# sebastianffx/stainlib

Hardware: AMD Instinct MI355X
Metric: 1024x1024 H&E tiles/sec normalized (Macenko) (higher is better)
Workload: dtype f32; 1 GPU; configs[1]: batch of 512 tiles 1024x1024x3 uint8 per GPU, Macenko transform (fit once outside the timed region), tiles resident in HBM; tiles_per_gpu=512, failed_tiles=0

## Files before the change

stainlib_amd/csrc/stats_finish.hpp:

```cpp
#pragma once
#include "stats_selection.hpp"
#include "stats_sweeps.hpp"

namespace sl {

struct SampleAngleKey {
    const uint32_t* sample; TabView tab; float V[6]; int cps_log2; int P; float ylimf;
    __device__ __forceinline__ float operator()(int b) const {
        if (sample_absent(b, cps_log2, P)) return nan_f();
        return of_word(sample[b]);
    }
    __device__ __forceinline__ float of_word(uint32_t s) const {
        const uint32_t r = s & 255u, g = (s >> 8) & 255u, bl = (s >> 16) & 255u;
        const bool tissue = is_tissue_f(tab.gam(r), tab.gam(g), tab.gam(bl), ylimf);
        const float k = angle_key(V, tab.odf(r), tab.odf(g), tab.odf(bl));
        return tissue ? k : nan_f();
    }
    __device__ __forceinline__ bool present(int b, int n_sample) const { return b < n_sample && !sample_absent(b, cps_log2, P); }
};
struct SampleConcKey {
    const uint32_t* sample; TabView tab; LassoK L; int cps_log2; int P; int col;
    __device__ __forceinline__ void both(int b, float& c1, float& c2) const {
        if (sample_absent(b, cps_log2, P)) { c1 = c2 = nan_f(); return; }
        of_word(sample[b], c1, c2);
// ... 100 lines not shown
    __syncthreads();
}

struct Census { uint32_t n_below, n_in, omin, omax; };
template <class KeyAt>
__device__ __noinline__ Census wg_bracket_census(int n, KeyAt key_at, float lo, float hi, SelScratch& S) {
    if (threadIdx.x == 0) { S.misc[4] = 0xffffffffu; S.misc[5] = 0; S.misc[6] = 0; S.misc[7] = 0; }
    __syncthreads();
    const uint32_t olo = f2ord(lo), ohi = f2ord(hi);
    uint32_t mn = 0xffffffffu, mx = 0, nb = 0, ni = 0;
    wg_for_each_key(n, key_at, [&](uint32_t o) {
        nb += o < olo ? 1u : 0u;
        if (o >= olo && o <= ohi) { ++ni; mn = min(mn, o); mx = max(mx, o); }
    });
    for (int o = 32; o > 0; o >>= 1) {
        mn = min(mn, (uint32_t)__shfl_xor((int)mn, o, 64));
        mx = max(mx, (uint32_t)__shfl_xor((int)mx, o, 64));
        nb += __shfl_xor((int)nb, o, 64);
        ni += __shfl_xor((int)ni, o, 64);
    }
    if ((threadIdx.x & 63) == 0) { atomicMin(&S.misc[4], mn); atomicMax(&S.misc[5], mx); atomicAdd(&S.misc[6], nb); atomicAdd(&S.misc[7], ni); }
    __syncthreads();
    const Census c{S.misc[6], S.misc[7], S.misc[4], S.misc[5]};
    __syncthreads();
    return c;
}

template <class TileKeyAt>
__device__ __forceinline__ void stage_order_stats(const float* cand, uint32_t n_in, uint32_t cap_list, bool complete, float lo, float hi,
                                                  long long lt, int P, const TileKeyAt& tile_key_at, uint32_t n,
                                                  long long k, float& xa, float& xb, int& fallbacks, SelScratch& S) {
    const long long k2 = (k + 1 < (long long)n) ? k + 1 : k;
    const bool covered = complete && k >= lt && k2 < lt + (long long)n_in;
    if (covered && lo == hi) {
        xa = xb = lo;
    } else if (covered && n_in <= cap_list) {
        wg_select_pair_small((int)n_in, CandKey{cand}, (uint32_t)(k - lt), xa, xb, S);
        if (k2 == k) xb = xa;
    } else {
        const Census c = wg_bracket_census(P, tile_key_at, lo, hi, S);
        if (c.n_in > 0 && c.omin == c.omax && k >= (long long)c.n_below && k2 < (long long)c.n_below + (long long)c.n_in) {
            xa = xb = ord2f(c.omin);
        } else {
            wg_select_pair(P, tile_key_at, (uint32_t)k, xa, xb, S);
            if (k2 == k) xb = xa;
        }
        fallbacks += 1;
    }
}

struct PickScale { float lo[2], sc[2]; };
__device__ __forceinline__ int pick_bin(float k, float lo, float sc) { return min(511, max(0, (int)((k - lo) * sc))); }

__device__ __forceinline__ void wg_pick2(const float* cand0, const float* cand1, const uint32_t* n_in, const bool* want, const uint32_t* krel,
                                         const PickScale& ps, float* xa , float* xb , bool* done , SelScratch& S) {
    const int tid = threadIdx.x, lane = tid & 63, wave = tid >> 6;
#pragma unroll
    for (int b = 0; b < 2; ++b)
        if (wave == b && want[b]) wave_locate(S.hist + 512 * b, 512, krel[b], &S.misc[16 + 3 * b], lane);
    if (tid < 2) { S.misc[24 + tid] = 0; S.misc[26 + tid] = 0xffffffffu; }
    __syncthreads();
    uint32_t bin[2], below[2], cnt[2];
#pragma unroll
    for (int b = 0; b < 2; ++b) { bin[b] = S.misc[16 + 3 * b]; below[b] = S.misc[17 + 3 * b]; cnt[b] = S.misc[18 + 3 * b]; done[b] = want[b] && cnt[b] <= 512u && cnt[b] > 0u; }
    __syncthreads();
    float* list = reinterpret_cast<float*>(S.hist);
#pragma unroll
    for (int b = 0; b < 2; ++b) {
        if (!done[b]) continue;
        const float* cand = b ? cand1 : cand0;
        const int n = (int)n_in[b];
        constexpr int U = 4;
        const int bd = blockDim.x;
        uint32_t best = 0xffffffffu;
        float kn[U];
#pragma unroll
        for (int u = 0; u < U; ++u) { const int i = tid + u * bd; kn[u] = as_global(cand)[i < n ? i : 0]; }
        for (int i0 = tid; i0 < n; i0 += U * bd) {
            float k[U];
#pragma unroll
            for (int u = 0; u < U; ++u) {
                k[u] = kn[u];
                const int i = i0 + (U + u) * bd;
                kn[u] = as_global(cand)[i < n ? i : 0];
            }
#pragma unroll
            for (int u = 0; u < U; ++u) {
                if (i0 + u * bd >= n) continue;
                const int kb = pick_bin(k[u], ps.lo[b], ps.sc[b]);
                if (kb == (int)bin[b]) { const uint32_t pos = atomicAdd(&S.misc[24 + b], 1u); if (pos < 512u) list[512 * b + pos] = k[u]; }
                else if (kb > (int)bin[b]) best = min(best, f2ord(k[u]));
            }
        }
        for (int o = 32; o > 0; o >>= 1) best = min(best, (uint32_t)__shfl_xor((int)best, o, 64));
        if (lane == 0 && best != 0xffffffffu) atomicMin(&S.misc[26 + b], best);
    }
    __syncthreads();
    if (tid < 4) S.misc[28 + tid] = 0;
    __syncthreads();
#pragma unroll
    for (int b = 0; b < 2; ++b) {
        if (!done[b]) continue;
        const uint32_t m = cnt[b], ra = krel[b] - below[b];
        if ((uint32_t)tid < m) {
            const float me = list[512 * b + tid];
            uint32_t r = 0;
            for (uint32_t j = 0; j < m; ++j) {
                const float o = list[512 * b + j];
                r += (o < me || (o == me && j < (uint32_t)tid)) ? 1u : 0u;
            }
            if (r == ra) S.misc[28 + 2 * b] = __float_as_uint(me);
            if (r == ra + 1) S.misc[29 + 2 * b] = __float_as_uint(me);
        }
    }
    __syncthreads();
#pragma unroll
    for (int b = 0; b < 2; ++b) {
        if (!done[b]) continue;
        xa[b] = __uint_as_float(S.misc[28 + 2 * b]);
        const bool same_bin = krel[b] - below[b] + 1 < cnt[b];
        const uint32_t nx = S.misc[26 + b];
        xb[b] = same_bin ? __uint_as_float(S.misc[29 + 2 * b]) : (nx != 0xffffffffu ? ord2f(nx) : xa[b]);
    }
    __syncthreads();
}

template <bool TWO_COLS, class TileKeyAt>
__device__ __forceinline__ void stage_pick2(const float* cand0, const float* cand1, const uint32_t* n_in, uint32_t cap_list, bool complete,
                                            const float* lo, const float* hi, const long long* lt, int P, TileKeyAt tile_key_at, uint32_t n,
                                            const long long* k, const PickScale& ps, float* res , int& fallbacks, SelScratch& S) {
    bool fast[2], has2[2];
    uint32_t krel[2];
#pragma unroll
    for (int b = 0; b < 2; ++b) {
        const long long k2 = (k[b] + 1 < (long long)n) ? k[b] + 1 : k[b];
        has2[b] = k2 != k[b];
        const bool covered = complete && k[b] >= lt[b] && k2 < lt[b] + (long long)n_in[b];
        fast[b] = covered && lo[b] < hi[b] && n_in[b] <= cap_list;
        krel[b] = fast[b] ? (uint32_t)(k[b] - lt[b]) : 0u;
    }
    float xa[2] = {0, 0}, xb[2] = {0, 0};
    bool done[2] = {false, false};
    if (fast[0] | fast[1]) wg_pick2(cand0, cand1, n_in, fast, krel, ps, xa, xb, done, S);
#pragma unroll
    for (int b = 0; b < 2; ++b) {
        if (done[b]) {
            if (!has2[b]) xb[b] = xa[b];
        } else {
            if constexpr (TWO_COLS) tile_key_at.col = b;
            stage_order_stats(b ? cand1 : cand0, n_in[b], cap_list, complete, lo[b], hi[b], lt[b], P, tile_key_at, n, k[b], xa[b], xb[b], fallbacks, S);
        }
        res[2 * b] = xa[b]; res[2 * b + 1] = xb[b];
    }
}

__device__ __noinline__ void raw_flush(uint32_t buf_lds, uint32_t n, uint32_t* dst, unsigned int* head, uint32_t cap) {
#if defined(__HIP_DEVICE_COMPILE__)
    SL_LDS const uint32_t* buf = (SL_LDS const uint32_t*)buf_lds;
#else
    const uint32_t* buf = nullptr;
#endif
    const int lane = threadIdx.x & 63;
    uint32_t base = 0;
    if (lane == 0) base = atomicAdd(head, n);
    base = __builtin_amdgcn_readfirstlane(base);
    for (uint32_t i = lane; i < n; i += 64)
        if (base + i < cap) as_global(dst)[base + i] = buf[i];
}

struct RawSink {
    uint32_t buf;
    uint32_t n;
    uint32_t* dst;
    unsigned int* head;
    unsigned int* overflow;
    uint32_t cap;
    uint32_t stage_cap;
    __device__ __forceinline__ void flush(int) {
        if (n != 0) raw_flush(buf, n, dst, head, cap);
        n = 0;
    }
    __device__ __forceinline__ void put(unsigned long long m, const Chunk& ch, int px, int lane) {
        put_value(m, chunk_pixel(ch, px) & 0xffffffu, lane);
    }
    __device__ __forceinline__ void put_value(unsigned long long m, uint32_t value, int lane) {
        const uint32_t cnt = (uint32_t)__popcll(m);
        if (__builtin_expect(n + cnt > stage_cap, 0)) flush(lane);
        const uint32_t rank = __builtin_amdgcn_mbcnt_hi((uint32_t)(m >> 32), __builtin_amdgcn_mbcnt_lo((uint32_t)m, 0u));
#if defined(__HIP_DEVICE_COMPILE__)
        uint32_t sbase;
        asm("s_lshl2_add_u32 %0, %1, %2" : "=s"(sbase) : "s"(n), "s"(buf) : "scc");
        const uint32_t addr = sbase + 4u * rank;
        unsigned long long saved;
        asm volatile("s_mov_b64 %0, exec\n\ts_mov_b64 exec, %1\n\tds_write_b32 %2, %3\n\ts_mov_b64 exec, %0"
                     : "=&s"(saved) : "s"(m), "v"(addr), "v"(value) : "memory");
#else
        (void)rank; (void)value;
#endif
        n += cnt;
    }
};


// ... 16 lines not shown
    __device__ __forceinline__ TabView view() const { return TabView{base, 8u, 4u, 0u}; }
};
__device__ __forceinline__ void fin_tab_build(RowTab& tab) {
    float2* p = reinterpret_cast<float2*>(tab.e);
    float2 e = make_float2(0.0f, 0.0f);
    if (threadIdx.x < 256) e = p[threadIdx.x * 32];
    __syncthreads();
    if (threadIdx.x < 256) p[threadIdx.x] = e;
    __syncthreads();
}

template <int NT>
__device__ __forceinline__ void fin_tab_expand(RowTab& tab) {
    float2* p = reinterpret_cast<float2*>(tab.e);
    constexpr int PER = 256 * 32 / NT;
    float2 e[PER];
#pragma unroll
    for (int j = 0; j < PER; ++j) e[j] = p[threadIdx.x / 32 + j * (NT / 32)];
    __syncthreads();
#pragma unroll
    for (int j = 0; j < PER; ++j) p[threadIdx.x + j * NT] = e[j];
    __syncthreads();
}

struct WordAngleKey {
    FinTab T; float V[6]; float ylimf;
    __device__ __forceinline__ void of_word(uint32_t s, float& k0, float& k1, bool& valid) const {
        const float2 er = T.gam_odf(T.addr(s, 0)), eg = T.gam_odf(T.addr(s, 1)), eb = T.gam_odf(T.addr(s, 2));
        valid = is_tissue_f(er.x, eg.x, eb.x, ylimf);
        k0 = k1 = angle_key(V, er.y, eg.y, eb.y);
    }
};
struct WordConcKey {
    FinTab T; LassoK L;
    __device__ __forceinline__ void of_word(uint32_t s, float& k0, float& k1, bool& valid) const {
        lasso2(L, T.odf(T.addr(s, 0)), T.odf(T.addr(s, 1)), T.odf(T.addr(s, 2)), k0, k1);
        valid = true;
    }
};

__device__ __forceinline__ void lds_count_masked(unsigned long long m, uint32_t addr, uint32_t one) {
#if defined(__HIP_DEVICE_COMPILE__)
    unsigned long long saved;
    asm volatile("s_mov_b64 %0, exec\n\ts_mov_b64 exec, %1\n\tds_add_u32 %2, %3\n\ts_mov_b64 exec, %0"
                 : "=&s"(saved) : "s"(m), "v"(addr), "v"(one) : "memory");
#else
    (void)m; (void)addr; (void)one;
#endif
}

struct RefineOut { uint32_t n_lt[2], n_in[2], n_valid; PickScale ps; };
template <class WordKey2>
__device__ __forceinline__ RefineOut wg_refine_s(const uint32_t* raw, int n_raw, const WordKey2& key2, float lo0, float hi0, float lo1, float hi1,
                                                 float* cand0, float* cand1, uint32_t cap_list, uint32_t stage_lds, uint32_t stage_entries,
                                                 SelScratch& S) {
    const int tid = threadIdx.x, lane = tid & 63;
    if (tid < 5) S.misc[8 + tid] = 0;
    for (int i = tid; i < 1024; i += blockDim.x) S.hist[i] = 0;
    RefineOut r;
    r.ps.lo[0] = lo0; r.ps.lo[1] = lo1;
    r.ps.sc[0] = (hi0 > lo0 && lo0 > -INFINITY && hi0 < INFINITY) ? 512.0f * 0.999999f / (hi0 - lo0) : 0.0f;
    r.ps.sc[1] = (hi1 > lo1 && lo1 > -INFINITY && hi1 < INFINITY) ? 512.0f * 0.999999f / (hi1 - lo1) : 0.0f;
    __syncthreads();
    stage_lds = (uint32_t)__builtin_amdgcn_readfirstlane((int)stage_lds);
    RawSink s0{stage_lds, 0u, reinterpret_cast<uint32_t*>(cand0), &S.misc[11], nullptr, cap_list, stage_entries};
    RawSink s1{stage_lds + 4u * stage_entries, 0u, reinterpret_cast<uint32_t*>(cand1), &S.misc[12], nullptr, cap_list, stage_entries};
    const float vlo0 = in_vgpr(lo0), vhi0 = in_vgpr(hi0), vlo1 = in_vgpr(lo1), vhi1 = in_vgpr(hi1);
    const float psl0 = in_vgpr(r.ps.lo[0]), psc0 = in_vgpr(r.ps.sc[0]), psl1 = in_vgpr(r.ps.lo[1]), psc1 = in_vgpr(r.ps.sc[1]);
    const uint32_t hist_lds = lds_address(S.hist);
    uint32_t one = 1u;
    asm("" : "+v"(one));
    uint32_t lt0 = 0, lt1 = 0, nv = 0;
    constexpr int U = 4;
    const int step = (int)blockDim.x * U;
    const int last = n_raw > 0 ? n_raw - 1 : 0;
    int i0 = (tid - lane) * U;
    uint32_t wn[U];
#pragma unroll
    for (int u = 0; u < U; ++u) wn[u] = as_global(raw)[min(i0 + u * 64 + lane, last)];
    for (; i0 < n_raw; i0 += step) {
        uint32_t w[U];
#pragma unroll
        for (int u = 0; u < U; ++u) {
            w[u] = wn[u];
            wn[u] = as_global(raw)[min(i0 + step + u * 64 + lane, last)];
        }
#pragma unroll
        for (int u = 0; u < U; ++u) {
            float k0, k1;
            bool valid;
            key2.of_word(w[u], k0, k1, valid);
            const bool inb = i0 + u * 64 + lane < n_raw;
            const unsigned long long mv = __builtin_amdgcn_ballot_w64(valid) & __builtin_amdgcn_ballot_w64(inb);
            const unsigned long long l0 = __builtin_amdgcn_ballot_w64(k0 < vlo0) & mv, l1 = __builtin_amdgcn_ballot_w64(k1 < vlo1) & mv;
            const unsigned long long m0 = __builtin_amdgcn_ballot_w64(k0 <= vhi0) & ~l0 & mv, m1 = __builtin_amdgcn_ballot_w64(k1 <= vhi1) & ~l1 & mv;
            nv += (uint32_t)__popcll(mv);
            lt0 += (uint32_t)__popcll(l0);
            lt1 += (uint32_t)__popcll(l1);
            lds_count_masked(m0, hist_lds + 4u * (uint32_t)pick_bin(k0, psl0, psc0), one);
            lds_count_masked(m1, hist_lds + 2048u + 4u * (uint32_t)pick_bin(k1, psl1, psc1), one);
            s0.put_value(m0, __float_as_uint(k0), lane);
            s1.put_value(m1, __float_as_uint(k1), lane);
        }
    }
    s0.flush(lane);
    s1.flush(lane);
    if (lane == 0) { if (nv) atomicAdd(&S.misc[8], nv); if (lt0) atomicAdd(&S.misc[9], lt0); if (lt1) atomicAdd(&S.misc[10], lt1); }
    __threadfence_block();
    __syncthreads();
    r.n_lt[0] = S.misc[9]; r.n_lt[1] = S.misc[10]; r.n_in[0] = S.misc[11]; r.n_in[1] = S.misc[12]; r.n_valid = S.misc[8];
    __syncthreads();
    return r;
}

constexpr float kBoxZ = 3.6f;
template <int THREADS>
__device__ __forceinline__ void angle_brackets(const SampleAngleKey& key, int n_sample, double pct, float* lo, float* hi,
                                               SelScratch& S, float* box = nullptr, float zs = 1.0f) {
    constexpr int KPT = kMaxSample / THREADS;
    uint32_t ord[1][KPT];
#ifdef SL_DEBUG_SUBCLK
    long long bclk_t_ = wall_clock64();
#endif
    static_assert(KPT % kBrkBatch == 0, "");
#pragma unroll
    for (int j0 = 0; j0 < KPT; j0 += kBrkBatch) {
        uint32_t w[kBrkBatch];
#pragma unroll
        for (int g = 0; g < kBrkBatch; ++g) {
            const int b = (j0 + g) * THREADS + (int)threadIdx.x;
            w[g] = b < n_sample ? as_global(key.sample)[b] : 0u;
        }
#pragma unroll
        for (int g = 0; g < kBrkBatch; ++g) {
            const int b = (j0 + g) * THREADS + (int)threadIdx.x;
            const float k = key.of_word(w[g]);
            ord[0][j0 + g] = (k == k && key.present(b, n_sample)) ? f2ord(k) : kAbsent;
        }
    }
    SL_BCLK(5);
    const int set_of[2] = {0, 0};
    const double p2[2] = {100.0 - pct, pct};
    wg_brackets_regs<1, KPT, 2>(ord, set_of, p2, lo, hi, S, kBracketZ * zs);
    if (box) {
        const bool closed = (lo[0] > -INFINITY) & (hi[0] < INFINITY) & (lo[1] > -INFINITY) & (hi[1] < INFINITY);
        if (closed) {
#pragma unroll
            for (int b = 0; b < 2; ++b) {
                const float m = 0.5f * (lo[b] + hi[b]), r = (float)kBoxFrac * 0.5f * (hi[b] - lo[b]);
                box[2 * b] = m - r; box[2 * b + 1] = m + r;
            }
        } else {
            const double n = (double)S.misc[6], q = p2[0] / 100.0;
            const bool inside = n > 0.0 && floor(q * (n - 1.0) - (double)(kBoxZ * zs) * sqrt(fmax(q * (1.0 - q) * n, 0.0))) - 1.0 >= 0.0;
            float blo[2] = {-INFINITY, -INFINITY}, bhi[2] = {INFINITY, INFINITY};
            __syncthreads();
            if (inside) wg_brackets_regs<1, KPT, 2>(ord, set_of, p2, blo, bhi, S, kBoxZ * zs);
            box[0] = blo[0]; box[1] = bhi[0]; box[2] = blo[1]; box[3] = bhi[1];
        }
    }
// ... 35 lines not shown
```

stainlib_amd/csrc/stats_fused.hpp:

```cpp
#pragma once
#include "stats_phase_kernels.hpp"
#include "stats_cube.hpp"
#include "stats_twosweep.hpp"

namespace sl {

struct FusedArgs {
    const uint8_t* rgb;
    uint8_t* out;
    int n_tiles;
    int P;
    int stride_log2;
    int n_sample;
    float ylimf;
    double lam;
    double pct;
    const double* M_tgt;
    const double* maxC_tgt;
    int cap_raw, cap_list;
    uint32_t* raw;
    int cap_ang;
    uint32_t* raw_ang;
    float* cand;
    uint32_t* sample;
// ... 274 lines not shown
    const int tid = threadIdx.x;
    const TabReaderB TB = TabReaderB::make_at(FusedLds<NT>::tab);
    const int nch = (P + 3) >> 2;
    ApplyK K;
    apply_consts(sh.M, sh.maxC, M_tgt, maxC_tgt, lam, K);
    int t, c0, c1;
    fused_geometry<NT>(nch, tid, t, c0, c1);
    if (c0 >= c1) return;
    if (stream) {
        if (K.fast) apply_sweep<ALIGNED, true, TabReaderB, true>(src, dst, P, c0, c1, t, kFusedThreads, TB, K);
        else apply_sweep<ALIGNED, false, TabReaderB, true>(src, dst, P, c0, c1, t, kFusedThreads, TB, K);
    } else {
        if (K.fast) apply_sweep<ALIGNED, true, TabReaderB, false>(src, dst, P, c0, c1, t, kFusedThreads, TB, K);
        else apply_sweep<ALIGNED, false, TabReaderB, false>(src, dst, P, c0, c1, t, kFusedThreads, TB, K);
    }
}

template <int NT, bool ALIGNED>
__device__ __noinline__ void fused_sweep2_cube(FusedShared<NT>* shp, const uint8_t* src_, uint32_t* rawl_, uint32_t* rawa_, int P_, int cap_raw_, int cap_ang_,
                                               float ylimf_, int stream_) {
    FusedShared<NT>& sh = *shp;
    const uint8_t* src = uni_ptr(src_);
    uint32_t* rawl = uni_ptr(rawl_);
    uint32_t* rawa = uni_ptr(rawa_);
    const int P = __builtin_amdgcn_readfirstlane(P_), cap_raw = __builtin_amdgcn_readfirstlane(cap_raw_), stream = __builtin_amdgcn_readfirstlane(stream_);
    const int cap_ang = __builtin_amdgcn_readfirstlane(cap_ang_);
    const float ylimf = uni(ylimf_);
    const int tid = threadIdx.x, wave = tid >> 6;
    const TabReaderB TB = TabReaderB::make_at(FusedLds<NT>::tab);
    const int nch = (P + 3) >> 2;
    SelConsts K;
    for (int i = 0; i < 6; ++i) K.V[i] = in_vgpr(sh.Vf[i]);
    K.L.g12 = 0.0f;
    K.xmin = -INFINITY;
#pragma unroll
    for (int i = 0; i < 2; ++i) {
        K.u[i][0] = in_vgpr(sh.mk.u[i][0]); K.u[i][1] = in_vgpr(sh.mk.u[i][1]); K.kt[i] = in_vgpr(sh.mk.kt[i]);
        K.eps[i] = in_vgpr(sh.mk.eps[i]); K.thr[i] = in_vgpr(sh.mk.thr[i]);
    }
    K.lo0 = uni(sh.lo[0]); K.hi0 = uni(sh.hi[0]); K.lo1 = uni(sh.lo[1]); K.hi1 = uni(sh.hi[1]);
    static_assert(offsetof(FusedShared<NT>, n_ang) == offsetof(FusedShared<NT>, n_raw) + 4 && offsetof(FusedShared<NT>, n_raw) % 8 == 0, "");
    const RawDirect direct{rawl, rawa, reinterpret_cast<unsigned long long*>(&sh.n_raw), (uint32_t)cap_raw, (uint32_t)cap_ang};
    static_assert(offsetof(FusedShared<NT>, S) % 4096 == 0 && offsetof(SelScratch, hist) == 0, "the cube mask must be 4 KB aligned");
    const uint32_t bits_lds = FusedLds<NT>::hist;
    const uint32_t ring_lds = (uint32_t)__builtin_amdgcn_readfirstlane((int)(FusedLds<NT>::stage + (uint32_t)wave * FusedLds<NT>::stage_wave));
    int t, c0, c1;
    fused_geometry<NT>(nch, tid, t, c0, c1);
    if (c0 >= c1) return;
    if (stream) select_sweep_cube<ALIGNED, kFusedTrip, true>(src, P, c0, c1, t, kFusedThreads, TB, ylimf, K, bits_lds, ring_lds, direct);
    else select_sweep_cube<ALIGNED, kFusedTrip, false>(src, P, c0, c1, t, kFusedThreads, TB, ylimf, K, bits_lds, ring_lds, direct);
}

template <int NT>
__device__ SL_FINISH_ATTR int fused_finish2(FusedShared<NT>* shp, const uint8_t* src_, uint32_t* rawl_, uint32_t* rawa_, float* cand0_, float* cand1_, int P_,
                                          int cap_raw_, int cap_ang_, int cap_list_, float ylimf_, double pct_, double lam_, long long* subclk_, int ts_ = 0) {
    FusedShared<NT>& sh = *shp;
    const uint8_t* src = uni_ptr(src_);
    uint32_t* rawl = uni_ptr(rawl_);
    uint32_t* rawa = uni_ptr(rawa_);
    const int cap_ang = __builtin_amdgcn_readfirstlane(cap_ang_);
    float* cand0 = uni_ptr(cand0_);
    float* cand1 = uni_ptr(cand1_);
    const int P = __builtin_amdgcn_readfirstlane(P_), cap_raw = __builtin_amdgcn_readfirstlane(cap_raw_), cap_list = __builtin_amdgcn_readfirstlane(cap_list_);
    const float ylimf = uni(ylimf_);
    const double pct = uni_d(pct_), lam = uni_d(lam_);
    long long* subclk = uni_ptr(subclk_);
    const int ts = __builtin_amdgcn_readfirstlane(ts_);
    const int tid = threadIdx.x, wave = tid >> 6;
    int fallbacks = 0;
#ifdef SL_DEBUG_SUBCLK
#define SL_SUB(j) { __syncthreads(); if (subclk && tid == 0) subclk[(j)] = wall_clock64(); }
#else
#define SL_SUB(j)
#endif
    (void)subclk;
    const uint32_t T = (uint32_t)sh.sum[0];
    long long k[2];
    double gfrac[2];
    percentile_pos((double)T, 100.0 - pct, k[0], gfrac[0]);
    percentile_pos((double)T, pct, k[1], gfrac[1]);
    fin_tab_build(sh.tab);
    const FinTab FT{FusedLds<NT>::tab};
    const uint32_t stage_lds = FusedLds<NT>::tab + kFinTabBytes + (uint32_t)wave * fin_stage_bytes(NT);
    const uint32_t stage_entries = fin_stage_bytes(NT) / 8u;
    AngleTileKey tkey;
    tkey.src = src; tkey.tab = FT.view(); tkey.ylimf = ylimf;
    WordAngleKey rkey;
    rkey.T = FT; rkey.ylimf = ylimf;
    for (int i = 0; i < 6; ++i) { tkey.V[i] = sh.Vf[i]; rkey.V[i] = sh.Vf[i]; }
    const bool complete = sh.n_raw <= (uint32_t)cap_raw && sh.overflow == 0;
    const uint32_t n_raw = sh.n_raw < (uint32_t)cap_raw ? sh.n_raw : (uint32_t)cap_raw;
    const bool split = rawa != nullptr;
    const bool complete_a = split ? sh.n_ang <= (uint32_t)cap_ang : complete;
    const uint32_t n_a = split ? (sh.n_ang < (uint32_t)cap_ang ? sh.n_ang : (uint32_t)cap_ang) : n_raw;
    const uint32_t* lista = split ? rawa : rawl;
    const float los[2] = {sh.lo[0], sh.lo[1]}, his[2] = {sh.hi[0], sh.hi[1]};
    SL_SUB(2);
    const RefineOut ra = wg_refine_s(lista, (int)n_a, rkey, los[0], his[0], los[1], his[1], cand0, cand1, (uint32_t)cap_list, stage_lds,
                                     stage_entries, sh.S);
    SL_SUB(3);
    {
        const long long lt[2] = {(long long)ra.n_lt[0], (long long)T - (long long)ra.n_valid + (long long)ra.n_lt[1]};
        if (ts) {
            bool covered = complete_a;
#pragma unroll
            for (int b = 0; b < 2; ++b) {
                const long long k2 = (k[b] + 1 < (long long)T) ? k[b] + 1 : k[b];
                covered = covered & (k[b] >= lt[b]) & (k2 < lt[b] + (long long)ra.n_in[b]) & (ra.n_in[b] <= (uint32_t)cap_list);
            }
            if (!covered) {
                fin_tab_expand<NT>(sh.tab);
                return -1;
            }
        }
        float res[4];
        stage_pick2<false>(cand0, cand1, ra.n_in, (uint32_t)cap_list, complete_a, los, his, lt, P, tkey, T, k, ra.ps, res, fallbacks, sh.S);
        if (tid == 0) { sh.res[0] = res[0]; sh.res[1] = res[1]; sh.res[2] = res[2]; sh.res[3] = res[3]; }
        __syncthreads();
    }
    SL_SUB(5);
    if (tid < 64) {
        double M[6];
        stain_matrix_from_angles(sh.Vd, sh.res, gfrac, M, tid);
        if (tid == 0) {
            for (int i = 0; i < 6; ++i) sh.M[i] = M[i];
            if (stain_matrix_singular(M)) sh.status = SL_TILE_DEGENERATE_COV;
            const bool use = sh.status == SL_TILE_OK && complete && merged_verify(sh.mk, M, lam);
            sh.conc_done = use ? 1 : 0;
            sh.why = use ? 0 : (!sh.mk.ok ? SL_RESWEEP_NO_BOX : (!complete ? SL_RESWEEP_LIST_FULL : SL_RESWEEP_OUTSIDE_BOX));
            if (use) { LassoK L; lasso_consts(M, lam, L); sh.L = L; }
        }
    }
    __syncthreads();
    SL_SUB(6);
    if (sh.conc_done) {
        long long kc;
        double gc;
        percentile_pos((double)P, 99.0, kc, gc);
        const long long kc2 = kc + 1 < (long long)P ? kc + 1 : kc;
        WordConcKey ckey2;
        ckey2.T = FT; ckey2.L = sh.L;
        const float cl[2] = {sh.mk.L[0], sh.mk.L[1]}, chh[2] = {sh.mk.H[0], sh.mk.H[1]};
        const RefineOut rc = wg_refine_s(rawl, (int)n_raw, ckey2, cl[0], chh[0], cl[1], chh[1], cand0, cand1, (uint32_t)cap_list,
                                         stage_lds, stage_entries, sh.S);
        SL_SUB(14);
#ifdef SL_DEBUG_SUBCLK
        if (subclk && tid == 0) {
            long long* q = subclk;
            q[8] = 100ll * n_a; q[9] = 100ll * n_raw; q[10] = 100ll * (ra.n_in[0] + ra.n_in[1]); q[11] = 100ll * (rc.n_in[0] + rc.n_in[1]);
        }
#endif
        const long long n_plain = (long long)P - (long long)sh.n_raw;
        const long long clt[2] = {n_plain + rc.n_lt[0], n_plain + rc.n_lt[1]};
        bool covered = true;
#pragma unroll
        for (int col = 0; col < 2; ++col)
            covered = covered & (kc >= clt[col]) & (kc2 < clt[col] + (long long)rc.n_in[col]) & (rc.n_in[col] <= (uint32_t)cap_list);
        if (covered) {
            ConcTileKey ctk;
            ctk.src = src; ctk.tab = FT.view(); ctk.L = sh.L; ctk.col = 0;
            const long long kk[2] = {kc, kc};
            float res[4];
            stage_pick2<true>(cand0, cand1, rc.n_in, (uint32_t)cap_list, true, cl, chh, clt, P, ctk, (uint32_t)P, kk, rc.ps, res, fallbacks, sh.S);
            if (tid == 0) {
                sh.maxC[0] = np_lerp((double)res[0], (double)res[1], gc);
                sh.maxC[1] = np_lerp((double)res[2], (double)res[3], gc);
                if (!(sh.maxC[0] > 0.0) || !(sh.maxC[1] > 0.0)) sh.status = SL_TILE_ZERO_MAXC;
            }
        } else if (tid == 0) {
            sh.conc_done = 0;
            sh.why = (rc.n_in[0] > (uint32_t)cap_list || rc.n_in[1] > (uint32_t)cap_list) ? SL_RESWEEP_LIST_FULL : SL_RESWEEP_BRACKET_MISSED;
        }
        __syncthreads();
        SL_SUB(15);
    }
    fin_tab_expand<NT>(sh.tab);
    return fallbacks;
#undef SL_SUB
}

template <int NT>
__device__ __noinline__ void phase0_estimate(FusedShared<NT>* shp, int mode_) {
    FusedShared<NT>& sh = *shp;
    const int mode = __builtin_amdgcn_readfirstlane(mode_);
    double Vd[6], wv[3];
    float Vf[6];
    const int st = eigvecs_from_moments(sh.sum, Vd, Vf, wv);
    const double ns = sh.sum[0];
    const double l1 = wv[0], l2 = wv[1], l3 = wv[2] > 0.0 ? wv[2] : 0.0;
    bool ok = st == SL_TILE_OK && ns >= (double)kTsMinTissue && l2 > 1e-9 * l1 && l2 - l3 > 0.05 * l2;
    double tau = 0.0;
    if (ok) {
        tau = kTiltZ * sqrt(kClusterDeff / ns) * fmax(sqrt(l3 * l2) / (l2 - l3), sqrt(l3 * l1) / (l1 - l3));
        tau = fmax(tau, kTsMinTau);
        ok = tau <= (mode >= 2 ? kTsMaxTau : kTsAutoMaxTau);
    }
    double nd[3] = {Vd[2] * Vd[5] - Vd[4] * Vd[3], Vd[4] * Vd[1] - Vd[0] * Vd[5], Vd[0] * Vd[3] - Vd[2] * Vd[1]};
    const double nn = 1.0 / sqrt(nd[0] * nd[0] + nd[1] * nd[1] + nd[2] * nd[2]);
    if (mode == 4 && ok) {
        double b[3];
        for (int c = 0; c < 3; ++c) b[c] = Vd[2 * c + 1] + 0.05 * nd[c] * nn;
        const double nb = 1.0 / sqrt(b[0] * b[0] + b[1] * b[1] + b[2] * b[2]);
        for (int c = 0; c < 3; ++c) { Vd[2 * c + 1] = b[c] * nb; Vf[2 * c + 1] = (float)Vd[2 * c + 1]; }
        nd[0] = Vd[2] * Vd[5] - Vd[4] * Vd[3]; nd[1] = Vd[4] * Vd[1] - Vd[0] * Vd[5]; nd[2] = Vd[0] * Vd[3] - Vd[2] * Vd[1];
    }
    const double nn2 = 1.0 / sqrt(nd[0] * nd[0] + nd[1] * nd[1] + nd[2] * nd[2]);
    for (int i = 0; i < 6; ++i) { sh.ts.Vd[i] = Vd[i]; sh.Vd[i] = Vd[i]; sh.Vf[i] = Vf[i]; }
    for (int c = 0; c < 3; ++c) { sh.ts.nd[c] = nd[c] * nn2; sh.ts.fn[c] = (float)(nd[c] * nn2); }
    sh.ts.tau = tau;
    sh.ts.gH[0] = l1 - l3; sh.ts.gH[1] = l2 - l3;
    sh.res[0] = (float)(4.0 * sqrt(l3));
    sh.res[1] = (float)(sh.sum[1] / ns); sh.res[2] = (float)(sh.sum[2] / ns); sh.res[3] = (float)(sh.sum[3] / ns);
    sh.status = ok ? SL_TILE_OK : SL_TILE_DEGENERATE_COV;
}

template <int NT>
// ... 337 lines not shown
        double t = 0;
        for (int p = 0; p < a.parts; ++p) t += a.partials[((size_t)tile * a.parts + p) * 10 + tid];
        sh.sum[tid] = t;
    }
    __syncthreads();
    if (tid == 0) {
        double Vd[6];
        float Vf[6];
        sh.status = eigvecs_from_moments(sh.sum, Vd, Vf);
        for (int i = 0; i < 6; ++i) { sh.Vd[i] = Vd[i]; sh.Vf[i] = Vf[i]; }
        sh.mk.ok = 0;
        sh.xmin = -INFINITY;
    }
    __syncthreads();
    if (sh.status == SL_TILE_OK)
        fused_finish1<kMFinishThreads>(&sh, a.sample + (size_t)tile * a.n_sample, a.n_sample, a.stride_log2, a.P, a.ylimf, a.pct, a.lam, nullptr, 0);
    __syncthreads();
    if (tid == 0) {
        st.status = sh.status;
        st.n_tissue = sh.sum[0];
        for (int i = 0; i < 6; ++i) { st.Vd[i] = sh.Vd[i]; st.Vf[i] = sh.Vf[i]; }
        st.lo[0] = sh.lo[0]; st.hi[0] = sh.hi[0]; st.lo[1] = sh.lo[1]; st.hi[1] = sh.hi[1];
        st.fallbacks = 0;
        st.n_raw = 0; st.overflow = 0;
        TileMerged& tm = a.mstate[tile];
        tm.mk = sh.mk;
        tm.xmin = sh.xmin;
        tm.conc_done = 0;
    }
}

static __global__ __launch_bounds__(kMFinishThreads) void k_finish2m(StatsArgs a, double* M_out, double* maxC_out, int32_t* status_out,
                                                                    int32_t* fallbacks_out, int tile0) {
    __shared__ FusedShared<kMFinishThreads> sh;
    fused_lds_origin(sh);
    const int tile = blockIdx.x, tid = threadIdx.x;
    TileState& st = a.state[tile];
    TileMerged& tm = a.mstate[tile];
    const bool bad = st.status != SL_TILE_OK;
    int fallbacks = 0;
    if (!bad) {
        sh.tab.fill_b();
        if (tid == 0) {
            sh.status = SL_TILE_OK;
            sh.sum[0] = st.n_tissue;
            for (int i = 0; i < 6; ++i) { sh.Vd[i] = st.Vd[i]; sh.Vf[i] = st.Vf[i]; }
            sh.lo[0] = st.lo[0]; sh.hi[0] = st.hi[0]; sh.lo[1] = st.lo[1]; sh.hi[1] = st.hi[1];
            sh.n_raw = st.n_raw; sh.overflow = st.overflow;
            sh.mk = tm.mk;
            sh.conc_done = 0;
            sh.maxC[0] = sh.maxC[1] = nan_d();
        }
        __syncthreads();
        fallbacks = fused_finish2<kMFinishThreads>(&sh, a.rgb + (size_t)tile * a.P * 3, a.raw + (size_t)tile * a.cap_raw, nullptr,
                                                   a.cand + ((size_t)tile * 2 + 0) * a.cap_list, a.cand + ((size_t)tile * 2 + 1) * a.cap_list, a.P,
                                                   a.cap_raw, 0, a.cap_list, a.ylimf, a.pct, a.lam, nullptr);
        __syncthreads();
        const bool singular = sh.status == SL_TILE_DEGENERATE_COV;
        const bool settled = sh.conc_done != 0 || singular;
        if (tid == 0) {
            st.status = sh.status;
            for (int i = 0; i < 6; ++i) st.M[i] = singular ? nan_d() : sh.M[i];
            st.maxC[0] = (singular || !sh.conc_done) ? nan_d() : sh.maxC[0];
            st.maxC[1] = (singular || !sh.conc_done) ? nan_d() : sh.maxC[1];
            st.fallbacks += fallbacks;
            st.n_raw = 0; st.overflow = 0;
            tm.conc_done = settled ? 1 : 0;
        }
        if (!settled) {
            if (tid == 0) { LassoK L; lasso_consts(sh.M, a.lam, L); sh.L = L; }
            __syncthreads();
            SampleConcKey ckey;
            ckey.sample = a.sample + (size_t)tile * a.n_sample; ckey.tab = view_of_b(sh.tab); ckey.L = sh.L; ckey.cps_log2 = a.stride_log2 - 2;
            ckey.P = a.P; ckey.col = 0;
            float lo[2], hi[2];
            conc_brackets<kMFinishThreads>(ckey, a.n_sample, lo, hi, sh.S);
            if (tid == 0) { st.lo[0] = lo[0]; st.hi[0] = hi[0]; st.lo[1] = lo[1]; st.hi[1] = hi[1]; }
            return;
        }
    } else if (tid == 0) {
        for (int i = 0; i < 6; ++i) st.M[i] = nan_d();
        st.maxC[0] = st.maxC[1] = nan_d();
        tm.conc_done = 1;
    }
    __syncthreads();
    if (tid < 6 && M_out) M_out[(size_t)(tile0 + tile) * 6 + tid] = st.M[tid];
    if (tid < 2 && maxC_out) maxC_out[(size_t)(tile0 + tile) * 2 + tid] = st.maxC[tid];
    if (tid == 0 && status_out) status_out[tile0 + tile] = st.status;
    if (tid == 0 && fallbacks_out) fallbacks_out[tile0 + tile] = bad ? 0 : st.fallbacks;
}

template <int NT, bool ALIGNED>
__device__ __noinline__ int fused_conc_resweep(FusedShared<NT>* shp, const uint8_t* src_, uint32_t* samp_, uint32_t* rawl_, float* cand0_, float* cand1_, int P_,
                                               int cap_raw_, int cap_list_, float ylimf_, double lam_, int stream_, int n_sample_, int stride_log2_,
                                               long long* clk_, long long* subclk_) {
    FusedShared<NT>& sh = *shp;
    const uint8_t* src = uni_ptr(src_);
    uint32_t* samp = uni_ptr(samp_);
    uint32_t* rawl = uni_ptr(rawl_);
    float* cand0 = uni_ptr(cand0_);
    float* cand1 = uni_ptr(cand1_);
    const int P = __builtin_amdgcn_readfirstlane(P_), cap_raw = __builtin_amdgcn_readfirstlane(cap_raw_), cap_list = __builtin_amdgcn_readfirstlane(cap_list_);
    const int stream = __builtin_amdgcn_readfirstlane(stream_), n_sample = __builtin_amdgcn_readfirstlane(n_sample_);
    const int stride_log2 = __builtin_amdgcn_readfirstlane(stride_log2_);
    const float ylimf = uni(ylimf_);
    const double lam = uni_d(lam_);
    long long* clk = uni_ptr(clk_);
    long long* subclk = uni_ptr(subclk_);
// ... 114 lines not shown
                sh.conc_done = 0;
                sh.use_cube = 0;
                sh.ts.ok = 0; sh.ts.why = kTsOff; sh.ts.dense = 0;
            }
            __syncthreads();
            const bool ts_try = a.two_sweep >= 2 || (a.two_sweep == 1 && ts_backoff == 0);
            if (ts_try) {
                fused_phase0<NT>(&sh, src, samp, a.P, a.cl_lines, a.ylimf, a.pct, a.lam, a.two_sweep, a.cap_raw, a.cap_ang, a.cap_list,
#ifdef SL_DEBUG_SUBCLK
                                 (a.phase_clock && a.debug_stop == -7) ? a.phase_clock + (size_t)a.n_tiles * 24 + (size_t)tile * 16 : nullptr
#else
                                 nullptr
#endif
                                 );
                __syncthreads();
            }
            const bool ts_on = sh.ts.ok != 0;
            if (a.two_sweep == 1) ts_backoff = ts_try ? (ts_on ? 0 : kTsBackoff) : ts_backoff - 1;
            if (ts_try) { SL_PHASE(4); }
            if (ts_on) fused_sweep1c<NT, ALIGNED>(&sh, src, rawl, rawa, a.P, a.cap_raw, a.cap_ang, a.ylimf, stream ? 1 : 0);
            else fused_sweep1<NT, ALIGNED>(&sh, src, samp, a.P, a.ylimf, a.stride_log2, stream ? 1 : 0);
            if (ts_on && lane_id() == 0) sh.ts.dense = 1;
            __threadfence_block();
            __syncthreads();
            if (lane_id() < 10) {
                double t = 0;
                for (int w = 0; w < NT / 64; ++w) t += sh.red[w][lane_id()];
                sh.sum[lane_id()] = t;
            }
            __syncthreads();
            SL_PHASE(1);
            SL_SUB(0);
            if (lane_id() == 0) {
                double Vd[6];
                float Vf[6];
                sh.status = eigvecs_from_moments(sh.sum, Vd, Vf);
                for (int i = 0; i < 6; ++i) { sh.Vd[i] = Vd[i]; sh.Vf[i] = Vf[i]; }
                sh.conc_done = 0;
            }
            __syncthreads();
            SL_SUB(1);
            bool direct = false;
            if (sh.status == SL_TILE_OK && ts_on) {
                if (lane_id() < 64) {
                    float br[4];
                    const bool okv = ts_verify(sh.ts, sh.Vd, br, lane_id(), a.two_sweep == 3);
                    if (lane_id() == 0) {
                        sh.lo[0] = br[0]; sh.hi[0] = br[1]; sh.lo[1] = br[2]; sh.hi[1] = br[3];
                        if (!okv) { sh.ts.ok = 0; sh.ts.why = kTsPlane; }
                    }
                }
                __syncthreads();
                if (sh.ts.ok) {
                    const int fb = fused_finish2<NT>(&sh, src, rawl, rawa, cand0, cand1, a.P, a.cap_raw, a.cap_ang, a.cap_list, a.ylimf, a.pct, a.lam,
#ifdef SL_DEBUG_SUBCLK
                                                     a.phase_clock ? a.phase_clock + (size_t)a.n_tiles * 8 + (size_t)tile * 16 : nullptr
#else
                                                     nullptr
#endif
                                                     , 1);
                    if (fb >= 0) { fallbacks += fb; direct = true; }
                    else if (lane_id() == 0) { sh.ts.ok = 0; sh.ts.why = kTsBracket; }
                }
                if (!direct) {
                    if (lane_id() == 0) {
                        sh.n_raw = 0; sh.n_ang = 0; sh.overflow = 0;
                        sh.conc_done = 0;
                        sh.use_cube = 0;
                    }
                    __syncthreads();
                }
                SL_PHASE(2);
                SL_PHASE(3);
            }
            if (sh.status == SL_TILE_OK && !direct) {
                fused_finish1<NT>(&sh, samp, ts_on ? a.cl_lines * kClusterPx : a.n_sample, ts_on ? -a.cl_scale_log2 : a.stride_log2, a.P, a.ylimf, a.pct, a.lam,
#ifdef SL_DEBUG_SUBCLK
                                  a.phase_clock ? a.phase_clock + (size_t)a.n_tiles * 8 + (size_t)tile * 16 : nullptr
#else
                                  nullptr
#endif
                                  , a.use_cube);
                SL_PHASE(2);
                run_select(true, src);
                SL_PHASE(3);
                fallbacks += fused_finish2<NT>(&sh, src, rawl, (sh.use_cube & 1) ? rawa : nullptr, cand0, cand1, a.P, a.cap_raw, a.cap_ang, a.cap_list, a.ylimf,
                                               a.pct, a.lam,
#ifdef SL_DEBUG_SUBCLK
                                               a.phase_clock ? a.phase_clock + (size_t)a.n_tiles * 8 + (size_t)tile * 16 : nullptr
#else
                                               nullptr
#endif
                                               );
            }
        } else {
            gather_sample<ALIGNED>(src, a.P, a.stride_log2, samp, a.n_sample, lane_id(), NT);
            if (lane_id() == 0) {
                dict_iter_init(sh.it);
                sh.n_raw = 0; sh.overflow = 0;
                sh.conc_done = 0;
            }
            __syncthreads();
            DictProgress pr{1, 0, 0, 0};
            if (stream) dict_learn<ALIGNED, NT, false, true>(src, a.P, nch, lane_id(), TB, a.ylimf, a.stride_log2, samp, a.n_sample, a.dl_lambda,
                                                             a.dl_tol, a.dl_max_sweeps, sh.it, sh.red, sh.sum, pr);
            else dict_learn<ALIGNED, NT, false, false>(src, a.P, nch, lane_id(), TB, a.ylimf, a.stride_log2, samp, a.n_sample, a.dl_lambda,
                                                       a.dl_tol, a.dl_max_sweeps, sh.it, sh.red, sh.sum, pr);
            sweeps_used = pr.sweeps_used;
            if (lane_id() == 0) {
                sh.status = sh.it.status;
                if (sh.status == SL_TILE_OK) {
                    dict_iter_stain_matrix(sh.it, sh.M);
                    if (stain_matrix_singular(sh.M)) sh.status = SL_TILE_DEGENERATE_COV;
                }
            }
        }
        __syncthreads();
        const bool bad = sh.status != SL_TILE_OK;
        const bool resweep = !bad && !sh.conc_done;
        if (resweep) {
            fallbacks += fused_conc_resweep<NT, ALIGNED>(&sh, src, samp, rawl, cand0, cand1, a.P, a.cap_raw, a.cap_list, a.ylimf, a.lam, stream ? 1 : 0,
                                                         (METHOD == kMethodMacenko && sh.ts.dense != 0) ? a.cl_lines * kClusterPx : a.n_sample,
                                                         (METHOD == kMethodMacenko && sh.ts.dense != 0) ? -1 : a.stride_log2,
#ifdef SL_DEVTOOLS
                                                         (METHOD == kMethodMacenko && a.phase_clock) ? a.phase_clock + (size_t)tile * 8 : nullptr,
#else
                                                         nullptr,
#endif
#ifdef SL_DEBUG_SUBCLK
                                                         a.phase_clock ? a.phase_clock + (size_t)a.n_tiles * 8 + (size_t)tile * 16 : nullptr
#else
                                                         nullptr
#endif
                                                         );
        } else if (bad && sh.status != SL_TILE_ZERO_MAXC && lane_id() == 0) {
            for (int i = 0; i < 6; ++i) sh.M[i] = nan_d();
            sh.maxC[0] = sh.maxC[1] = nan_d();
        }
        __syncthreads();
// ... 38 lines not shown
```

Before: 364,700 tiles/s.

## Drop candidate list materialization; recompute keys from raw words during pick

The refine pass no longer writes in-bracket candidate keys to per-tile global cand buffers through LDS staging. It now only counts members per column. The pick stage re-reads the raw sample words and recomputes both keys per word, filtering by the bracket, and handles both columns in one fused pass. This removes global writes, staging and flushes, at the cost of re-reading the full raw list and redoing key evaluation, which includes a lasso solve for the concentration keys. The slow fallback now passes a null candidate list with zero capacity.

```diff
diff --git a/stainlib_amd/csrc/stats_finish.hpp b/stainlib_amd/csrc/stats_finish.hpp
--- a/stainlib_amd/csrc/stats_finish.hpp
+++ b/stainlib_amd/csrc/stats_finish.hpp
@@ -176,8 +176,24 @@
 struct PickScale { float lo[2], sc[2]; };
 __device__ __forceinline__ int pick_bin(float k, float lo, float sc) { return min(511, max(0, (int)((k - lo) * sc))); }
 
-__device__ __forceinline__ void wg_pick2(const float* cand0, const float* cand1, const uint32_t* n_in, const bool* want, const uint32_t* krel,
-                                         const PickScale& ps, float* xa , float* xb , bool* done , SelScratch& S) {
+__device__ __forceinline__ bool pick_member(bool valid, float k, float lo, float hi) { return valid && !(k < lo) && k <= hi; }
+
+template <class WordKey2>
+struct RawMemberKey {
+    const uint32_t* raw; WordKey2 key2; int b; float lo, hi;
+    __device__ __forceinline__ float operator()(int i) const {
+        float k0, k1;
+        bool valid;
+        key2.of_word(as_global(raw)[i], k0, k1, valid);
+        const float k = b ? k1 : k0;
+        return pick_member(valid, k, lo, hi) ? k : nan_f();
+    }
+};
+
+template <class WordKey2>
+__device__ __forceinline__ void wg_pick2(const uint32_t* raw, int n_raw, const WordKey2& key2, const float* lo, const float* hi,
+                                         const bool* want, const uint32_t* krel, const PickScale& ps, float* xa , float* xb ,
+                                         bool* done , SelScratch& S) {
     const int tid = threadIdx.x, lane = tid & 63, wave = tid >> 6;
 #pragma unroll
     for (int b = 0; b < 2; ++b)
@@ -189,35 +205,43 @@
     for (int b = 0; b < 2; ++b) { bin[b] = S.misc[16 + 3 * b]; below[b] = S.misc[17 + 3 * b]; cnt[b] = S.misc[18 + 3 * b]; done[b] = want[b] && cnt[b] <= 512u && cnt[b] > 0u; }
     __syncthreads();
     float* list = reinterpret_cast<float*>(S.hist);
-#pragma unroll
-    for (int b = 0; b < 2; ++b) {
-        if (!done[b]) continue;
-        const float* cand = b ? cand1 : cand0;
-        const int n = (int)n_in[b];
+    if (done[0] | done[1]) {
+        uint32_t best[2] = {0xffffffffu, 0xffffffffu};
         constexpr int U = 4;
-        const int bd = blockDim.x;
-        uint32_t best = 0xffffffffu;
-        float kn[U];
-#pragma unroll
-        for (int u = 0; u < U; ++u) { const int i = tid + u * bd; kn[u] = as_global(cand)[i < n ? i : 0]; }
-        for (int i0 = tid; i0 < n; i0 += U * bd) {
-            float k[U];
+        const int step = (int)blockDim.x * U;
+        const int last = n_raw > 0 ? n_raw - 1 : 0;
+        int i0 = (tid - lane) * U;
+        uint32_t wn[U];
+#pragma unroll
+        for (int u = 0; u < U; ++u) wn[u] = as_global(raw)[min(i0 + u * 64 + lane, last)];
+        for (; i0 < n_raw; i0 += step) {
+            uint32_t w[U];
 #pragma unroll
             for (int u = 0; u < U; ++u) {
-                k[u] = kn[u];
-                const int i = i0 + (U + u) * bd;
-                kn[u] = as_global(cand)[i < n ? i : 0];
+                w[u] = wn[u];
+                wn[u] = as_global(raw)[min(i0 + step + u * 64 + lane, last)];
             }
 #pragma unroll
             for (int u = 0; u < U; ++u) {
-                if (i0 + u * bd >= n) continue;
-                const int kb = pick_bin(k[u], ps.lo[b], ps.sc[b]);
-                if (kb == (int)bin[b]) { const uint32_t pos = atomicAdd(&S.misc[24 + b], 1u); if (pos < 512u) list[512 * b + pos] = k[u]; }
-                else if (kb > (int)bin[b]) best = min(best, f2ord(k[u]));
+                float k[2];
+                bool valid;
+                key2.of_word(w[u], k[0], k[1], valid);
+                valid = valid && i0 + u * 64 + lane < n_raw;
+#pragma unroll
+                for (int b = 0; b < 2; ++b) {
+                    if (!done[b] || !pick_member(valid, k[b], lo[b], hi[b])) continue;
+                    const int kb = pick_bin(k[b], ps.lo[b], ps.sc[b]);
+                    if (kb == (int)bin[b]) { const uint32_t pos = atomicAdd(&S.misc[24 + b], 1u); if (pos < 512u) list[512 * b + pos] = k[b]; }
+                    else if (kb > (int)bin[b]) best[b] = min(best[b], f2ord(k[b]));
+                }
             }
         }
-        for (int o = 32; o > 0; o >>= 1) best = min(best, (uint32_t)__shfl_xor((int)best, o, 64));
-        if (lane == 0 && best != 0xffffffffu) atomicMin(&S.misc[26 + b], best);
+#pragma unroll
+        for (int b = 0; b < 2; ++b) {
+            if (!done[b]) continue;
+            for (int o = 32; o > 0; o >>= 1) best[b] = min(best[b], (uint32_t)__shfl_xor((int)best[b], o, 64));
+            if (lane == 0 && best[b] != 0xffffffffu) atomicMin(&S.misc[26 + b], best[b]);
+        }
     }
     __syncthreads();
     if (tid < 4) S.misc[28 + tid] = 0;
@@ -249,8 +273,8 @@
     __syncthreads();
 }
 
-template <bool TWO_COLS, class TileKeyAt>
-__device__ __forceinline__ void stage_pick2(const float* cand0, const float* cand1, const uint32_t* n_in, uint32_t cap_list, bool complete,
+template <bool TWO_COLS, class WordKey2, class TileKeyAt>
+__device__ __forceinline__ void stage_pick2(const uint32_t* raw, int n_raw, const WordKey2& key2, const uint32_t* n_in, uint32_t cap_list, bool complete,
                                             const float* lo, const float* hi, const long long* lt, int P, TileKeyAt tile_key_at, uint32_t n,
                                             const long long* k, const PickScale& ps, float* res , int& fallbacks, SelScratch& S) {
     bool fast[2], has2[2];
@@ -265,14 +289,17 @@
     }
     float xa[2] = {0, 0}, xb[2] = {0, 0};
     bool done[2] = {false, false};
-    if (fast[0] | fast[1]) wg_pick2(cand0, cand1, n_in, fast, krel, ps, xa, xb, done, S);
+    if (fast[0] | fast[1]) wg_pick2(raw, n_raw, key2, lo, hi, fast, krel, ps, xa, xb, done, S);
 #pragma unroll
     for (int b = 0; b < 2; ++b) {
         if (done[b]) {
             if (!has2[b]) xb[b] = xa[b];
+        } else if (fast[b]) {
+            wg_select_pair_small(n_raw, RawMemberKey<WordKey2>{raw, key2, b, lo[b], hi[b]}, krel[b], xa[b], xb[b], S);
+            if (!has2[b]) xb[b] = xa[b];
         } else {
             if constexpr (TWO_COLS) tile_key_at.col = b;
-            stage_order_stats(b ? cand1 : cand0, n_in[b], cap_list, complete, lo[b], hi[b], lt[b], P, tile_key_at, n, k[b], xa[b], xb[b], fallbacks, S);
+            stage_order_stats(nullptr, n_in[b], 0u, complete, lo[b], hi[b], lt[b], P, tile_key_at, n, k[b], xa[b], xb[b], fallbacks, S);
         }
         res[2 * b] = xa[b]; res[2 * b + 1] = xb[b];
     }
@@ -395,7 +422,6 @@
 struct RefineOut { uint32_t n_lt[2], n_in[2], n_valid; PickScale ps; };
 template <class WordKey2>
 __device__ __forceinline__ RefineOut wg_refine_s(const uint32_t* raw, int n_raw, const WordKey2& key2, float lo0, float hi0, float lo1, float hi1,
-                                                 float* cand0, float* cand1, uint32_t cap_list, uint32_t stage_lds, uint32_t stage_entries,
                                                  SelScratch& S) {
     const int tid = threadIdx.x, lane = tid & 63;
     if (tid < 5) S.misc[8 + tid] = 0;
@@ -405,15 +431,12 @@
     r.ps.sc[0] = (hi0 > lo0 && lo0 > -INFINITY && hi0 < INFINITY) ? 512.0f * 0.999999f / (hi0 - lo0) : 0.0f;
     r.ps.sc[1] = (hi1 > lo1 && lo1 > -INFINITY && hi1 < INFINITY) ? 512.0f * 0.999999f / (hi1 - lo1) : 0.0f;
     __syncthreads();
-    stage_lds = (uint32_t)__builtin_amdgcn_readfirstlane((int)stage_lds);
-    RawSink s0{stage_lds, 0u, reinterpret_cast<uint32_t*>(cand0), &S.misc[11], nullptr, cap_list, stage_entries};
-    RawSink s1{stage_lds + 4u * stage_entries, 0u, reinterpret_cast<uint32_t*>(cand1), &S.misc[12], nullptr, cap_list, stage_entries};
     const float vlo0 = in_vgpr(lo0), vhi0 = in_vgpr(hi0), vlo1 = in_vgpr(lo1), vhi1 = in_vgpr(hi1);
     const float psl0 = in_vgpr(r.ps.lo[0]), psc0 = in_vgpr(r.ps.sc[0]), psl1 = in_vgpr(r.ps.lo[1]), psc1 = in_vgpr(r.ps.sc[1]);
     const uint32_t hist_lds = lds_address(S.hist);
     uint32_t one = 1u;
     asm("" : "+v"(one));
-    uint32_t lt0 = 0, lt1 = 0, nv = 0;
+    uint32_t lt0 = 0, lt1 = 0, in0 = 0, in1 = 0, nv = 0;
     constexpr int U = 4;
     const int step = (int)blockDim.x * U;
     const int last = n_raw > 0 ? n_raw - 1 : 0;
@@ -440,15 +463,19 @@
             nv += (uint32_t)__popcll(mv);
             lt0 += (uint32_t)__popcll(l0);
             lt1 += (uint32_t)__popcll(l1);
+            in0 += (uint32_t)__popcll(m0);
+            in1 += (uint32_t)__popcll(m1);
             lds_count_masked(m0, hist_lds + 4u * (uint32_t)pick_bin(k0, psl0, psc0), one);
             lds_count_masked(m1, hist_lds + 2048u + 4u * (uint32_t)pick_bin(k1, psl1, psc1), one);
-            s0.put_value(m0, __float_as_uint(k0), lane);
-            s1.put_value(m1, __float_as_uint(k1), lane);
-        }
-    }
-    s0.flush(lane);
-    s1.flush(lane);
-    if (lane == 0) { if (nv) atomicAdd(&S.misc[8], nv); if (lt0) atomicAdd(&S.misc[9], lt0); if (lt1) atomicAdd(&S.misc[10], lt1); }
+        }
+    }
+    if (lane == 0) {
+        if (nv) atomicAdd(&S.misc[8], nv);
+        if (lt0) atomicAdd(&S.misc[9], lt0);
+        if (lt1) atomicAdd(&S.misc[10], lt1);
+        if (in0) atomicAdd(&S.misc[11], in0);
+        if (in1) atomicAdd(&S.misc[12], in1);
+    }
     __threadfence_block();
     __syncthreads();
     r.n_lt[0] = S.misc[9]; r.n_lt[1] = S.misc[10]; r.n_in[0] = S.misc[11]; r.n_in[1] = S.misc[12]; r.n_valid = S.misc[8];
diff --git a/stainlib_amd/csrc/stats_fused.hpp b/stainlib_amd/csrc/stats_fused.hpp
--- a/stainlib_amd/csrc/stats_fused.hpp
+++ b/stainlib_amd/csrc/stats_fused.hpp
@@ -350,21 +350,19 @@
 }
 
 template <int NT>
-__device__ SL_FINISH_ATTR int fused_finish2(FusedShared<NT>* shp, const uint8_t* src_, uint32_t* rawl_, uint32_t* rawa_, float* cand0_, float* cand1_, int P_,
-                                          int cap_raw_, int cap_ang_, int cap_list_, float ylimf_, double pct_, double lam_, long long* subclk_, int ts_ = 0) {
+__device__ SL_FINISH_ATTR int fused_finish2(FusedShared<NT>* shp, const uint8_t* src_, uint32_t* rawl_, uint32_t* rawa_, int P_, int cap_raw_,
+                                          int cap_ang_, int cap_list_, float ylimf_, double pct_, double lam_, long long* subclk_, int ts_ = 0) {
     FusedShared<NT>& sh = *shp;
     const uint8_t* src = uni_ptr(src_);
     uint32_t* rawl = uni_ptr(rawl_);
     uint32_t* rawa = uni_ptr(rawa_);
     const int cap_ang = __builtin_amdgcn_readfirstlane(cap_ang_);
-    float* cand0 = uni_ptr(cand0_);
-    float* cand1 = uni_ptr(cand1_);
     const int P = __builtin_amdgcn_readfirstlane(P_), cap_raw = __builtin_amdgcn_readfirstlane(cap_raw_), cap_list = __builtin_amdgcn_readfirstlane(cap_list_);
     const float ylimf = uni(ylimf_);
     const double pct = uni_d(pct_), lam = uni_d(lam_);
     long long* subclk = uni_ptr(subclk_);
     const int ts = __builtin_amdgcn_readfirstlane(ts_);
-    const int tid = threadIdx.x, wave = tid >> 6;
+    const int tid = threadIdx.x;
     int fallbacks = 0;
 #ifdef SL_DEBUG_SUBCLK
 #define SL_SUB(j) { __syncthreads(); if (subclk && tid == 0) subclk[(j)] = wall_clock64(); }
@@ -379,8 +377,6 @@
     percentile_pos((double)T, pct, k[1], gfrac[1]);
     fin_tab_build(sh.tab);
     const FinTab FT{FusedLds<NT>::tab};
-    const uint32_t stage_lds = FusedLds<NT>::tab + kFinTabBytes + (uint32_t)wave * fin_stage_bytes(NT);
-    const uint32_t stage_entries = fin_stage_bytes(NT) / 8u;
     AngleTileKey tkey;
     tkey.src = src; tkey.tab = FT.view(); tkey.ylimf = ylimf;
     WordAngleKey rkey;
@@ -394,8 +390,7 @@
     const uint32_t* lista = split ? rawa : rawl;
     const float los[2] = {sh.lo[0], sh.lo[1]}, his[2] = {sh.hi[0], sh.hi[1]};
     SL_SUB(2);
-    const RefineOut ra = wg_refine_s(lista, (int)n_a, rkey, los[0], his[0], los[1], his[1], cand0, cand1, (uint32_t)cap_list, stage_lds,
-                                     stage_entries, sh.S);
+    const RefineOut ra = wg_refine_s(lista, (int)n_a, rkey, los[0], his[0], los[1], his[1], sh.S);
     SL_SUB(3);
     {
         const long long lt[2] = {(long long)ra.n_lt[0], (long long)T - (long long)ra.n_valid + (long long)ra.n_lt[1]};
@@ -412,7 +407,7 @@
             }
         }
         float res[4];
-        stage_pick2<false>(cand0, cand1, ra.n_in, (uint32_t)cap_list, complete_a, los, his, lt, P, tkey, T, k, ra.ps, res, fallbacks, sh.S);
+        stage_pick2<false>(lista, (int)n_a, rkey, ra.n_in, (uint32_t)cap_list, complete_a, los, his, lt, P, tkey, T, k, ra.ps, res, fallbacks, sh.S);
         if (tid == 0) { sh.res[0] = res[0]; sh.res[1] = res[1]; sh.res[2] = res[2]; sh.res[3] = res[3]; }
         __syncthreads();
     }
@@ -439,8 +434,7 @@
         WordConcKey ckey2;
         ckey2.T = FT; ckey2.L = sh.L;
         const float cl[2] = {sh.mk.L[0], sh.mk.L[1]}, chh[2] = {sh.mk.H[0], sh.mk.H[1]};
-        const RefineOut rc = wg_refine_s(rawl, (int)n_raw, ckey2, cl[0], chh[0], cl[1], chh[1], cand0, cand1, (uint32_t)cap_list,
-                                         stage_lds, stage_entries, sh.S);
+        const RefineOut rc = wg_refine_s(rawl, (int)n_raw, ckey2, cl[0], chh[0], cl[1], chh[1], sh.S);
         SL_SUB(14);
 #ifdef SL_DEBUG_SUBCLK
         if (subclk && tid == 0) {
@@ -459,7 +453,7 @@
             ctk.src = src; ctk.tab = FT.view(); ctk.L = sh.L; ctk.col = 0;
             const long long kk[2] = {kc, kc};
             float res[4];
-            stage_pick2<true>(cand0, cand1, rc.n_in, (uint32_t)cap_list, true, cl, chh, clt, P, ctk, (uint32_t)P, kk, rc.ps, res, fallbacks, sh.S);
+            stage_pick2<true>(rawl, (int)n_raw, ckey2, rc.n_in, (uint32_t)cap_list, true, cl, chh, clt, P, ctk, (uint32_t)P, kk, rc.ps, res, fallbacks, sh.S);
             if (tid == 0) {
                 sh.maxC[0] = np_lerp((double)res[0], (double)res[1], gc);
                 sh.maxC[1] = np_lerp((double)res[2], (double)res[3], gc);
@@ -903,8 +897,7 @@
             sh.maxC[0] = sh.maxC[1] = nan_d();
         }
         __syncthreads();
-        fallbacks = fused_finish2<kMFinishThreads>(&sh, a.rgb + (size_t)tile * a.P * 3, a.raw + (size_t)tile * a.cap_raw, nullptr,
-                                                   a.cand + ((size_t)tile * 2 + 0) * a.cap_list, a.cand + ((size_t)tile * 2 + 1) * a.cap_list, a.P,
+        fallbacks = fused_finish2<kMFinishThreads>(&sh, a.rgb + (size_t)tile * a.P * 3, a.raw + (size_t)tile * a.cap_raw, nullptr, a.P,
                                                    a.cap_raw, 0, a.cap_list, a.ylimf, a.pct, a.lam, nullptr);
         __syncthreads();
         const bool singular = sh.status == SL_TILE_DEGENERATE_COV;
@@ -1125,7 +1118,7 @@
                 }
                 __syncthreads();
                 if (sh.ts.ok) {
-                    const int fb = fused_finish2<NT>(&sh, src, rawl, rawa, cand0, cand1, a.P, a.cap_raw, a.cap_ang, a.cap_list, a.ylimf, a.pct, a.lam,
+                    const int fb = fused_finish2<NT>(&sh, src, rawl, rawa, a.P, a.cap_raw, a.cap_ang, a.cap_list, a.ylimf, a.pct, a.lam,
 #ifdef SL_DEBUG_SUBCLK
                                                      a.phase_clock ? a.phase_clock + (size_t)a.n_tiles * 8 + (size_t)tile * 16 : nullptr
 #else
@@ -1157,7 +1150,7 @@
                 SL_PHASE(2);
                 run_select(true, src);
                 SL_PHASE(3);
-                fallbacks += fused_finish2<NT>(&sh, src, rawl, (sh.use_cube & 1) ? rawa : nullptr, cand0, cand1, a.P, a.cap_raw, a.cap_ang, a.cap_list, a.ylimf,
+                fallbacks += fused_finish2<NT>(&sh, src, rawl, (sh.use_cube & 1) ? rawa : nullptr, a.P, a.cap_raw, a.cap_ang, a.cap_list, a.ylimf,
                                                a.pct, a.lam,
 #ifdef SL_DEBUG_SUBCLK
                                                a.phase_clock ? a.phase_clock + (size_t)a.n_tiles * 8 + (size_t)tile * 16 : nullptr
```

After: 365,500 tiles/s (median of 4 runs). About the same (+0.2%).
